# visinf/irr

Measured on AMD Instinct MI355X. Metric: image-pairs/sec fwd+bwd IRR-PWC 384x448 bs32, higher is better.
Workload: dtype f32 (fp16x2 split operands)

## Files before the change

### irr_amd/csrc/conv_x3.hip

```cpp
#include "x3_split.h"
#include "pack.h"
#include "amax.h"
#include <stdlib.h>
#include <atomic>

#ifdef X3S_TRACE
static unsigned long long* g_x3s_dbg = nullptr;
#endif

#ifndef X3_ABL
#define X3_ABL 0
#endif

int irr_amax_channels_launch(const float* x, int B, int C, long hw, long bs, float* out, hipStream_t st, bool zero);

namespace {

constexpr uint32_t OOB = 0x80000000u;

struct X3Args {
  const float* x;
  const u32x4* wq;
  const float* bias;
  const float* res;
  float* y;
  int B, Cin, H, W, Cout;
  int dil;
  int RD;
  int CoT, nchunk;
  int TR, TC, tiles_x, tiles_y;
  long x_bs, y_bs, res_bs;
  int lrelu, accumulate;
  float alpha;
  const float* mask;
  long mask_bs;
  int nmask;
  int ngy;
  int ksplit;
  float* part;
  const float* x_amax;
  int n_amax;
  float* y_amax;
  float* y_chmax;
  unsigned int* kcnt;
};

template <int CT, int PG, int NT, int PLANE_PIX, int NP = 3>
__global__ __launch_bounds__(CT* PG * 64, 2) void conv_x3_kernel(const X3Args a) {
  constexpr int NTHR = CT * PG * 64;
  constexpr int NR = (2 * PLANE_PIX + NTHR - 1) / NTHR;
  __shared__ u32x4 lds[2 * NP * PLANE_PIX];

  const int tid = threadIdx.x;
  const int lane = tid & 63;
  const int wave = __builtin_amdgcn_readfirstlane(tid >> 6);
  const int ct = wave % CT, pg = wave / CT;
  const int j = lane & 31, g = lane >> 5;
  const unsigned xpos = irr_xcd_order(blockIdx.x, gridDim.x);
  const int by = (int)(xpos % (unsigned)a.ngy);
  int bt = (int)(xpos / (unsigned)a.ngy);
  const int tx = bt % a.tiles_x;
  bt /= a.tiles_x;
  const int ty = bt % a.tiles_y;
  bt /= a.tiles_y;
  const int rr = bt % a.RD;
  const int b = bt / a.RD;
  const int y0 = ty * a.TR, x0 = tx * a.TC;
  const int d = a.dil;
  const int dy = a.RD > 1 ? 1 : d;
  const int Hs = (a.H - rr + a.RD - 1) / a.RD;
  const int LW = a.TC + 2 * d, LH = a.TR + 2 * dy;
  const int npix = LH * LW;
  const long hw = (long)a.H * a.W;
  const int cot = by * CT + ct;
  const bool active = cot < a.CoT;

  const __amdgpu_buffer_rsrc_t xr = __builtin_amdgcn_make_buffer_rsrc((void*)a.x, (short)0, (int)0x80000000u, 0x00020000);
  const __amdgpu_buffer_rsrc_t wr = __builtin_amdgcn_make_buffer_rsrc((void*)a.wq, (short)0, (int)0xffffffffu, 0x00020000);

  uint32_t svoff[NR];
  int swidx[NR];
#pragma unroll
  for (int r = 0; r < NR; ++r) {
    const int u = r * NTHR + tid;
    const int gg = u >= npix ? 1 : 0;
    const int pix = u - gg * npix;
    const bool inr = u < 2 * npix;
    const int ly = pix / LW, lx = pix - ly * LW;
    const int iy = y0 - dy + ly, ix = x0 - d + lx;
    const bool ok = inr && iy >= 0 && iy < Hs && ix >= 0 && ix < a.W;
    svoff[r] = ok ? (uint32_t)(((long)b * a.x_bs + (long)gg * 8 * hw + (long)(rr + iy * a.RD) * a.W + ix) * 4) : OOB;
    swidx[r] = inr ? gg * PLANE_PIX + pix : -1;
  }
  const uint32_t hw4 = (uint32_t)(hw * 4);
  const int tail_base = a.Cin - 16;

  int xidx[NT];
#pragma unroll
  for (int s = 0; s < NT; ++s) {
    const int t = (pg * NT + s) * 32 + j;
    const int row = t / a.TC, col = t - row * a.TC;
    xidx[s] = g * PLANE_PIX + row * LW + col;
  }
  const uint32_t wvoff = (uint32_t)((cot * 64 + lane) * 16);
  const uint32_t wpiece = (uint32_t)a.CoT * 1024u;
  const uint32_t wtap = (uint32_t)NP * wpiece;
  float sx = 1.f, inv_x = 1.f, inv_w = 1.f;
  if (NP == 2) {
    const int ex = x3_h2_exp(x3_h2_amax(a.x_amax, a.n_amax));
    const int ew = ((const int*)(a.wq + (long)a.nchunk * 9 * NP * a.CoT * 64))[0];
    sx = ldexpf(1.f, ex);
    inv_x = ldexpf(1.f, -ex);
    inv_w = ldexpf(1.f, -ew);
  }

  f32x16 acc[NT];
#pragma unroll
  for (int s = 0; s < NT; ++s)
#pragma unroll
    for (int r = 0; r < 16; ++r) acc[s][r] = 0.f;

  float raw[NR][8];
  auto issue_x = [&](int c) {
    const int ch0 = X3_ABL == 12 ? 0 : (c == a.nchunk - 1) ? tail_base : c * 16;
    const uint32_t s0 = (uint32_t)ch0 * hw4;
#pragma unroll
    for (int r = 0; r < NR; ++r)
#pragma unroll
      for (int e = 0; e < 8; ++e)
        raw[r][e] = (X3_ABL == 3 && c > 0) ? 1.f : __builtin_bit_cast(float, __builtin_amdgcn_raw_buffer_load_b32(xr, (int)svoff[r], (int)(s0 + e * hw4), 0));
  };
  u32x4 wa[2][NP];
  auto issue_w = [&](int slot, int c, int tap) {
    const uint32_t so = ((uint32_t)c * 9u + (uint32_t)tap) * wtap;
#pragma unroll
    for (int p = 0; p < NP; ++p)
      wa[slot][p] = __builtin_bit_cast(u32x4, __builtin_amdgcn_raw_buffer_load_b128(wr, (int)wvoff, (int)(so + p * wpiece), 0));
  };
  const int c_begin = (int)(((long)blockIdx.z * a.nchunk) / a.ksplit), c_end = (int)(((long)(blockIdx.z + 1) * a.nchunk) / a.ksplit);
  if (active) issue_w(0, c_begin, 0);

  for (int c = c_begin; c < c_end; ++c) {
    issue_x(c);
#pragma unroll
    for (int r = 0; r < NR; ++r) {
      u32x4 h, m, l;
      if (NP == 2) split8_h2<true>(raw[r], sx, h, m);
      else split8(raw[r], h, m, l);
      if (swidx[r] >= 0) {
        lds[swidx[r]] = h;
        lds[swidx[r] + 2 * PLANE_PIX] = m;
        if (NP == 3) lds[swidx[r] + 4 * PLANE_PIX] = l;
      }
    }
    __syncthreads();
    const bool more = c + 1 < c_end;
    if (active) {
#pragma unroll
      for (int tap = 0; tap < 9; ++tap) {
        const int slot = tap & 1;
        if (X3_ABL != 1) {
          const int nt = tap == 8 ? 0 : tap + 1;
          const int nc = tap == 8 ? (more ? c + 1 : c) : c;
          issue_w(slot ^ 1, nc, nt);
        }
        __builtin_amdgcn_sched_barrier(0);
        const int toff = (tap / 3) * LW * dy + (tap % 3) * d;
        u32x4 wdn;
        if (NP == 2) wdn = h2_hi_down(wa[slot][0]);
        u32x4 xb[2][NP];
#pragma unroll
        for (int p = 0; p < NP; ++p) xb[0][p] = lds[xidx[0] + toff + 2 * p * PLANE_PIX];
#pragma unroll
        for (int s = 0; s < NT; ++s) {
          const int cur = s & 1;
          if (s + 1 < NT) {
#pragma unroll
            for (int p = 0; p < NP; ++p) xb[cur ^ 1][p] = lds[xidx[s + 1] + toff + 2 * p * PLANE_PIX];
          }
          __builtin_amdgcn_sched_barrier(0);
          f32x16 t = acc[s];
          if constexpr (NP == 2) {
            t = mma_h(wa[slot][1], xb[cur][0], t);
            t = mma_h(wdn, xb[cur][1], t);
            t = mma_h(wa[slot][0], xb[cur][0], t);
          } else {
            if (X3_ABL != 20) {
            t = mma(wa[slot][NP - 1], xb[cur][0], t);
            t = mma(wa[slot][0], xb[cur][NP - 1], t);
            t = mma(wa[slot][1], xb[cur][1], t);
            }
            t = mma(wa[slot][1], xb[cur][0], t);
            t = mma(wa[slot][0], xb[cur][1], t);
            t = mma(wa[slot][0], xb[cur][0], t);
          }
          acc[s] = t;
          __builtin_amdgcn_sched_barrier(0);
        }
      }
#pragma unroll
      for (int p = 0; p < NP; ++p) wa[0][p] = wa[1][p];
    }
    __syncthreads();
  }
  if constexpr (NT > 4) {
    if (!active) return;
  }
  if (active && NP == 2) {
#pragma unroll
    for (int s = 0; s < NT; ++s)
#pragma unroll
      for (int r = 0; r < 16; ++r) acc[s][r] = (acc[s][r] * inv_x) * inv_w;
  }
  const long ohw = hw;
  bool split_out = a.ksplit > 1;
  if constexpr (NT <= 4)
  if (a.ksplit > 1 && a.kcnt != nullptr) {
    if (active) {
#pragma unroll
      for (int s = 0; s < NT; ++s) {
        const int t = (pg * NT + s) * 32 + j;
        const int row = t / a.TC, col = t - row * a.TC;
        const int oys = y0 + row, ox = x0 + col;
        if (oys >= Hs || ox >= a.W) continue;
        float* pb = a.part + (((long)blockIdx.z * a.B + b) * a.Cout) * ohw + (long)(rr + oys * a.RD) * a.W + ox;
#pragma unroll
        for (int r = 0; r < 16; ++r) {
          const int co = cot * 32 + (r & 3) + 8 * (r >> 2) + 4 * g;
          if (co < a.Cout) __hip_atomic_store(pb + (long)co * ohw, acc[s][r], __ATOMIC_RELAXED, __HIP_MEMORY_SCOPE_AGENT);
        }
      }
    }
    __shared__ unsigned int s_last;
    asm volatile("s_waitcnt vmcnt(0)" ::: "memory");
    __syncthreads();
    if (tid == 0) {
      const unsigned int old = atomicInc(a.kcnt + blockIdx.x, (unsigned int)a.ksplit - 1u);
      s_last = old == (unsigned int)a.ksplit - 1u ? 1u : 0u;
    }
    __syncthreads();
    if (!s_last) return;
    if (active) {
#pragma unroll
      for (int s = 0; s < NT; ++s) {
        const int t = (pg * NT + s) * 32 + j;
        const int row = t / a.TC, col = t - row * a.TC;
        const int oys = y0 + row, ox = x0 + col;
        if (oys >= Hs || ox >= a.W) continue;
        const long pofs0 = ((long)b * a.Cout) * ohw + (long)(rr + oys * a.RD) * a.W + ox;
        const long kstride = (long)a.B * a.Cout * ohw;
        f32x16 sum;
#pragma unroll
        for (int r = 0; r < 16; ++r) sum[r] = 0.f;
        for (int k = 0; k < a.ksplit; ++k) {
          float tv[16];
#pragma unroll
          for (int r = 0; r < 16; ++r) {
            const int co = cot * 32 + (r & 3) + 8 * (r >> 2) + 4 * g;
            const int cc = co < a.Cout ? co : a.Cout - 1;
            tv[r] = __hip_atomic_load(a.part + pofs0 + (long)cc * ohw + (long)k * kstride, __ATOMIC_RELAXED, __HIP_MEMORY_SCOPE_AGENT);
          }
#pragma unroll
          for (int r = 0; r < 16; ++r) sum[r] += tv[r];
        }
        acc[s] = sum;
      }
    }
    split_out = false;
  }
  if (!active) return;
  float ymax = 0.f;
  const bool want_amax = NP == 2 && a.y_amax != nullptr && !split_out;
  const bool want_ch = NP == 2 && a.y_chmax != nullptr && !split_out;
  float chm[16];
#pragma unroll
  for (int r = 0; r < 16; ++r) chm[r] = 0.f;

  const __amdgpu_buffer_rsrc_t yr = __builtin_amdgcn_make_buffer_rsrc((void*)(a.y + (long)b * a.y_bs), (short)0, (int)0x80000000u, 0x00020000);
  const __amdgpu_buffer_rsrc_t rsr =
      __builtin_amdgcn_make_buffer_rsrc((void*)(a.res ? a.res + (long)b * a.res_bs : a.y), (short)0, (int)0x80000000u, 0x00020000);
  const __amdgpu_buffer_rsrc_t mkr =
      __builtin_amdgcn_make_buffer_rsrc((void*)(a.mask ? a.mask + (long)b * a.mask_bs : a.y), (short)0, (int)0x80000000u, 0x00020000);
#pragma unroll
  for (int s = 0; s < NT; ++s) {
    const int t = (pg * NT + s) * 32 + j;
    const int row = t / a.TC, col = t - row * a.TC;
    const int oys = y0 + row, ox = x0 + col;
    if (oys >= Hs || ox >= a.W) continue;
    const long pofs = (long)(rr + oys * a.RD) * a.W + ox;
    if (split_out) {
      float* pb = a.part + (((long)blockIdx.z * a.B + b) * a.Cout) * ohw + pofs;
#pragma unroll
      for (int r = 0; r < 16; ++r) {
        const int co = cot * 32 + (r & 3) + 8 * (r >> 2) + 4 * g;
        if (co < a.Cout) pb[(long)co * ohw] = acc[s][r];
      }
      continue;
    }
    constexpr int RB = NT >= 8 ? 8 : 16;
#pragma unroll
    for (int r0 = 0; r0 < 16; r0 += RB) {
      uint32_t vo[RB];
      float bv[RB];
#pragma unroll
      for (int k = 0; k < RB; ++k) {
        const int r = r0 + k;
        const int co = cot * 32 + (r & 3) + 8 * (r >> 2) + 4 * g;
        const bool ok = co < a.Cout;
        vo[k] = ok ? (uint32_t)(((long)co * ohw + pofs) * 4) : OOB;
        bv[k] = (ok && a.bias) ? a.bias[co] : 0.f;
      }
      if (!a.res && !a.accumulate && !a.mask) {
#pragma unroll
        for (int k = 0; k < RB; ++k) {
          float v = acc[s][r0 + k] + bv[k];
          if (a.lrelu) v = irr_lrelu(v);
          v *= a.alpha;
          if (want_ch) { if (vo[k] != OOB) chm[r0 + k] = x3_amax_fold(chm[r0 + k], v); }
          else if (want_amax && vo[k] != OOB) ymax = x3_amax_fold(ymax, v);
          __builtin_amdgcn_raw_buffer_store_b32(__builtin_bit_cast(uint32_t, v), yr, (int)vo[k], 0, 0);
        }
        continue;
      }
      float rv[RB], dv[RB], mv[RB];
#pragma unroll
      for (int k = 0; k < RB; ++k) {
        const int r = r0 + k;
        const int co = cot * 32 + (r & 3) + 8 * (r >> 2) + 4 * g;
        rv[k] = __builtin_bit_cast(float, __builtin_amdgcn_raw_buffer_load_b32(rsr, (int)(a.res ? vo[k] : OOB), 0, 0));
        dv[k] = __builtin_bit_cast(float, __builtin_amdgcn_raw_buffer_load_b32(yr, (int)(a.accumulate ? vo[k] : OOB), 0, 0));
        mv[k] = __builtin_bit_cast(float, __builtin_amdgcn_raw_buffer_load_b32(mkr, (int)((a.mask && co < a.nmask) ? vo[k] : OOB), 0, 0));
      }
#pragma unroll
      for (int k = 0; k < RB; ++k) {
        const int r = r0 + k;
        const int co = cot * 32 + (r & 3) + 8 * (r >> 2) + 4 * g;
        float v = acc[s][r] + bv[k];
        if (a.lrelu) v = irr_lrelu(v);
        v = a.res ? rv[k] + a.alpha * v : v * a.alpha;
        v += dv[k];
        if (a.mask && co < a.nmask) v *= irr_lrelu_grad(mv[k]);
        if (want_ch) { if (vo[k] != OOB) chm[r] = x3_amax_fold(chm[r], v); }
        else if (want_amax && vo[k] != OOB) ymax = x3_amax_fold(ymax, v);
        __builtin_amdgcn_raw_buffer_store_b32(__builtin_bit_cast(uint32_t, v), yr, (int)vo[k], 0, 0);
      }
    }
  }
  if (want_ch && want_amax) {
#pragma unroll
    for (int r = 0; r < 16; ++r) ymax = __builtin_bit_cast(float, max(__builtin_bit_cast(uint32_t, ymax), __builtin_bit_cast(uint32_t, chm[r])));
  }
  if (want_amax) x3_amax_publish(ymax, a.y_amax);
  if (want_ch) {
    uint32_t mine = 0u;
#pragma unroll
    for (int r = 0; r < 16; ++r) {
      const uint32_t mb = x3_amax_half_upper(__builtin_bit_cast(uint32_t, chm[r]));
      mine = j == 16 + r ? mb : mine;
    }
    if (j >= 16) {
      const int r = j - 16;
      const int co = cot * 32 + (r & 3) + 8 * (r >> 2) + 4 * g;
      if (co < a.Cout) x3_amax_commit(__builtin_bit_cast(float, mine), a.y_chmax + co);
    }
  }
}

static thread_local float* g_next_chmax = nullptr;
static std::atomic<int> g_min_blocks{384};

struct X3SArgs {
  const float* x;
  const u32x4* wq;
  const float* bias;
  const float* res;
  float* y;
  int B, Cin, H, W, Cout;
  int tiles_x, tiles_y;
  long ntiles;
  long x_bs, y_bs, res_bs;
  int lrelu, accumulate;
  float alpha;
  const float* mask;
  long mask_bs;
  int nmask;
  unsigned long long* dbg;
  int wCoT, wcot;
  float* y2;
  long y2_bs;
  const float* x_amax;
  int n_amax;
  float* y_amax;
  float* y_chmax;
  const uint32_t* mask_bits;
  uint32_t* bits_out;
  long bits_tile0;
};

#ifdef X3S_TRACE
#define TR(slot) do { if (blockIdx.x == 7 && lane == 0 && ntr < 400) { dbgp[ntr++] = ((unsigned long long)(slot) << 56) | (__builtin_amdgcn_s_memtime() & 0xffffffffffffffull); } } while (0)
#else
#define TR(slot) do {} while (0)
#endif

#ifndef X3S_PRODUCERS_OLD
#define X3S_PRODUCERS_OLD 1
#endif
template <int EPI, int NP = 3>
__global__ __launch_bounds__(512) void conv_x3s_kernel(const X3SArgs a) {
  constexpr int PLANE_PIX = 352;
  constexpr int CHUNK = 2 * NP * PLANE_PIX;
  constexpr int LW = 34;
  constexpr int WUNITS = 18 * NP * 64;
  extern __shared__ u32x4 lds[];
  u32x4* const wl = lds;
  u32x4* const xl = lds + WUNITS;
  float* const ol = (float*)(lds + WUNITS + 2 * CHUNK);

  const int tid = threadIdx.x;
  const int lane = tid & 63;
  const int wave = __builtin_amdgcn_readfirstlane(tid >> 6);
  const long hw = (long)a.H * a.W;
  const long t_begin = irr_xcd_order(blockIdx.x, gridDim.x), t_step = gridDim.x;
#ifdef X3S_TRACE
  int ntr = 0;
  unsigned long long* dbgp = a.dbg + (size_t)wave * 400;
#endif

  for (int u = tid; u < WUNITS; u += 512) wl[u] = a.wq[((long)(u >> 6) * a.wCoT + a.wcot) * 64 + (u & 63)];
  float sx = 1.f, inv_x = 1.f, inv_w = 1.f;
  if (NP == 2) {
    const int ex = x3_h2_exp(x3_h2_amax(a.x_amax, a.n_amax));
    const int ew = ((const int*)(a.wq + (long)18 * NP * a.wCoT * 64))[0];
    sx = ldexpf(1.f, ex);
    inv_x = ldexpf(1.f, -ex);
    inv_w = ldexpf(1.f, -ew);
  }
  __syncthreads();

  if (X3S_PRODUCERS_OLD ? wave < 4 : wave >= 4) {
    const int ptid = X3S_PRODUCERS_OLD ? tid : tid - 256;
    const __amdgpu_buffer_rsrc_t xr = __builtin_amdgcn_make_buffer_rsrc((void*)a.x, (short)0, (int)0x80000000u, 0x00020000);
    const __amdgpu_buffer_rsrc_t rres = __builtin_amdgcn_make_buffer_rsrc((void*)a.res, (short)0, (int)0x80000000u, 0x00020000);
    const __amdgpu_buffer_rsrc_t ry = __builtin_amdgcn_make_buffer_rsrc((void*)a.y, (short)0, (int)0x80000000u, 0x00020000);
    const __amdgpu_buffer_rsrc_t rmask = __builtin_amdgcn_make_buffer_rsrc((void*)a.mask, (short)0, (int)0x80000000u, 0x00020000);
    const __amdgpu_buffer_rsrc_t ry2 = __builtin_amdgcn_make_buffer_rsrc((void*)(EPI == 3 ? a.y2 : a.y), (short)0, (int)0x80000000u, 0x00020000);
    const __amdgpu_buffer_rsrc_t rbits = __builtin_amdgcn_make_buffer_rsrc((void*)(EPI == 4 ? (const void*)a.mask_bits : (const void*)a.bits_out),
                                                                            (short)0, (int)0x80000000u, 0x00020000);
    const int su_gg = ptid / 100, su_rest = ptid % 100;
    const int su_ly = su_rest / 10, su_q = su_rest % 10;
    const bool su_act = ptid < 200;
    const uint32_t hw4 = (uint32_t)(hw * 4);
    const uint32_t c1off = (uint32_t)(a.Cin - 16) * hw4;
    f32x4 raw[2][8];
    struct TileAt { int b, ty, tx; };
    const int step_x = (int)(t_step % a.tiles_x), step_y = (int)((t_step / a.tiles_x) % a.tiles_y),
              step_b = (int)(t_step / ((long)a.tiles_x * a.tiles_y));
    auto advance = [&](TileAt& c) {
      c.tx += step_x;
      const int cx = c.tx >= a.tiles_x;
      c.tx -= cx ? a.tiles_x : 0;
      c.ty += step_y + cx;
      const int cy = c.ty >= a.tiles_y;
      c.ty -= cy ? a.tiles_y : 0;
      c.b += step_b + cy;
    };
    auto issue_chunk = [&](const TileAt& at, int c, bool valid) {
      const int tx = X3_ABL == 11 ? 1 : at.tx, ty = X3_ABL == 11 ? 1 : at.ty, b = X3_ABL == 11 ? 0 : at.b;
      const int iy = ty * 8 - 1 + su_ly, ix = tx * 32 - 4 + su_q * 4;
      const bool ok = valid && su_act && iy >= 0 && iy < a.H && ix >= 0 && ix < a.W && X3_ABL != 10;
      const uint32_t vo = ok ? (uint32_t)(((long)b * a.x_bs + (long)su_gg * 8 * hw + (long)iy * a.W + ix) * 4) : OOB;
#pragma unroll
      for (int e = 0; e < 8; ++e)
        raw[c][e] = __builtin_bit_cast(f32x4, __builtin_amdgcn_raw_buffer_load_b128(xr, (int)vo, (int)((c ? c1off : 0u) + e * hw4), 0));
    };
    auto write_chunk = [&](int c) {
      u32x4* buf = xl + c * CHUNK + su_gg * PLANE_PIX + su_ly * LW;
#pragma unroll
      for (int px = 0; px < 4; ++px) {
        const int lx = su_q * 4 + px - 3;
        float v[8];
#pragma unroll
        for (int e = 0; e < 8; ++e) v[e] = raw[c][e][px];
        u32x4 h, m, l;
        if (NP == 2) split8_h2<true>(v, sx, h, m);
        else split8(v, h, m, l);
        if (su_act && lx >= 0 && lx < LW) {
          buf[lx] = h;
          buf[lx + 2 * PLANE_PIX] = m;
          if (NP == 3) buf[lx + 4 * PLANE_PIX] = l;
        }
      }
    };
    const int eq_q = ptid & 7, eq_row = (ptid >> 3) & 7, eq_c8 = ptid >> 6;
    float bias_r[8];
#pragma unroll
    for (int e = 0; e < 8; ++e) bias_r[e] = (a.bias && eq_c8 * 8 + e < a.Cout) ? a.bias[eq_c8 * 8 + e] : 0.f;
    f32x4 erv[8], edv[8], emv[8];
    uint32_t evd = OOB, evd2 = OOB;
    uint32_t ebits = 0, ebo = OOB;
    auto epilogue_loads = [&](const TileAt& at, bool valid, long tix) {
      const int tx = at.tx, ty = at.ty, b = at.b;
      const int oy = ty * 8 + eq_row, ox = tx * 32 + eq_q * 4;
      const bool pv = valid && oy < a.H && ox < a.W;
      const long pofs = (long)oy * a.W + ox + (long)eq_c8 * 8 * hw;
      const uint32_t vr = (EPI >= 1 && pv && a.res) ? (uint32_t)(((long)b * a.res_bs + pofs) * 4) : OOB;
// ... 786 lines not shown
```

Before: 211.6.

## Double-buffer LDS input planes and interleave next-chunk loads with MFMA taps

Adds a pipelined path for the fp16x2 (NP==2), large-NT conv_x3 configurations. The LDS input plane is double-buffered, and loading, splitting and storing the next channel chunk are spread across the tap/subtile MFMA loop. This removes one barrier per chunk and hides the global load latency behind compute. Weight prefetch deepens to three slots, two taps ahead. The cost is double the LDS footprint and more live registers, which may lower occupancy or cause spills.

```diff
diff --git a/irr_amd/csrc/conv_x3.hip b/irr_amd/csrc/conv_x3.hip
--- a/irr_amd/csrc/conv_x3.hip
+++ b/irr_amd/csrc/conv_x3.hip
@@ -10,6 +10,9 @@
 
 #ifndef X3_ABL
 #define X3_ABL 0
+#endif
+#ifndef X3_PIPE
+#define X3_PIPE 1
 #endif
 
 int irr_amax_channels_launch(const float* x, int B, int C, long hw, long bs, float* out, hipStream_t st, bool zero);
@@ -49,7 +52,9 @@
 __global__ __launch_bounds__(CT* PG * 64, 2) void conv_x3_kernel(const X3Args a) {
   constexpr int NTHR = CT * PG * 64;
   constexpr int NR = (2 * PLANE_PIX + NTHR - 1) / NTHR;
-  __shared__ u32x4 lds[2 * NP * PLANE_PIX];
+  constexpr bool PIPE = X3_PIPE && X3_ABL != 13 && NP == 2 && NT >= 7 && NR <= 5;
+  constexpr int BUF = 2 * NP * PLANE_PIX;
+  __shared__ u32x4 lds[(PIPE ? 2 : 1) * BUF];
 
   const int tid = threadIdx.x;
   const int lane = tid & 63;
@@ -138,9 +143,112 @@
       wa[slot][p] = __builtin_bit_cast(u32x4, __builtin_amdgcn_raw_buffer_load_b128(wr, (int)wvoff, (int)(so + p * wpiece), 0));
   };
   const int c_begin = (int)(((long)blockIdx.z * a.nchunk) / a.ksplit), c_end = (int)(((long)(blockIdx.z + 1) * a.nchunk) / a.ksplit);
-  if (active) issue_w(0, c_begin, 0);
-
+  if (active && !PIPE) issue_w(0, c_begin, 0);
+
+  if constexpr (PIPE) {
+    constexpr auto XI = [](int r) { return NR <= 3 ? 3 * r : 2 * r; };
+    constexpr int XK = NR <= 3 ? 3 : 2;
+    u32x4 wp[3][NP];
+    auto issue_wp = [&](int slot, int c, int tap) {
+      const uint32_t so = ((uint32_t)c * 9u + (uint32_t)tap) * wtap;
+#pragma unroll
+      for (int p = 0; p < NP; ++p)
+        wp[slot][p] = __builtin_bit_cast(u32x4, __builtin_amdgcn_raw_buffer_load_b128(wr, (int)wvoff, (int)(so + p * wpiece), 0));
+    };
+    auto issue_round = [&](float (&v)[8], int c, int r, bool valid) {
+      const int ch0 = X3_ABL == 12 ? 0 : (c == a.nchunk - 1) ? tail_base : c * 16;
+      const uint32_t s0 = (uint32_t)ch0 * hw4;
+      const uint32_t vo = valid ? svoff[r] : OOB;
+#pragma unroll
+      for (int e = 0; e < 8; ++e)
+        v[e] = __builtin_bit_cast(float, __builtin_amdgcn_raw_buffer_load_b32(xr, (int)vo, (int)(s0 + e * hw4), 0));
+    };
+    auto write_round = [&](const u32x4& h, const u32x4& m, int r, int base) {
+      if (swidx[r] >= 0) {
+        lds[base + swidx[r]] = h;
+        lds[base + swidx[r] + 2 * PLANE_PIX] = m;
+      }
+    };
+    issue_x(c_begin);
+#pragma unroll
+    for (int r = 0; r < NR; ++r) {
+      u32x4 h, m;
+      split8_h2<true>(raw[r], sx, h, m);
+      write_round(h, m, r, 0);
+    }
+    __syncthreads();
+    if (!active) {
+      for (int c = c_begin; c + 1 < c_end; ++c) {
+        const int wb = ((c - c_begin) & 1) ? 0 : BUF;
+#pragma unroll
+        for (int r = 0; r < NR; ++r) {
+          float v[8];
+          u32x4 h, m;
+          issue_round(v, c + 1, r, true);
+          split8_h2<true>(v, sx, h, m);
+          write_round(h, m, r, wb);
+        }
+        __syncthreads();
+      }
+      return;
+    }
+    issue_wp(0, c_begin, 0);
+    issue_wp(1, c_begin, 1);
+    float v[8];
+    u32x4 sh, sm;
+    for (int c = c_begin; c < c_end; ++c) {
+      const bool more = c + 1 < c_end;
+      const int rb = ((c - c_begin) & 1) ? BUF : 0;
+      const int wb = BUF - rb;
+      const int cn = more ? c + 1 : c;
+#pragma unroll
+      for (int tap = 0; tap < 9; ++tap) {
+        const int slot = tap % 3;
+        if (X3_ABL != 1) {
+          const int nt = tap + 2 > 8 ? tap + 2 - 9 : tap + 2;
+          const int nc = tap + 2 > 8 ? (more ? c + 1 : c) : c;
+          issue_wp((tap + 2) % 3, nc, nt);
+        }
+        __builtin_amdgcn_sched_barrier(0);
+        const int toff = rb + (tap / 3) * LW * dy + (tap % 3) * d;
+        u32x4 wdn = h2_hi_down(wp[slot][0]);
+        u32x4 xb[2][NP];
+#pragma unroll
+        for (int p = 0; p < NP; ++p) xb[0][p] = lds[xidx[0] + toff + 2 * p * PLANE_PIX];
+#pragma unroll
+        for (int s = 0; s < NT; ++s) {
+          const int cur = s & 1;
+          if (s + 1 < NT) {
+#pragma unroll
+            for (int p = 0; p < NP; ++p) xb[cur ^ 1][p] = lds[xidx[s + 1] + toff + 2 * p * PLANE_PIX];
+          }
+          __builtin_amdgcn_sched_barrier(0);
+          f32x16 t = acc[s];
+          t = mma_h(wp[slot][1], xb[cur][0], t);
+          t = mma_h(wdn, xb[cur][1], t);
+          t = mma_h(wp[slot][0], xb[cur][0], t);
+          acc[s] = t;
+#pragma unroll
+          for (int r = 0; r < NR; ++r) {
+            if (s == 0 && XI(r) + XK == tap) split8_h2<true>(v, sx, sh, sm);
+            if (s == 0 && XI(r) == tap) issue_round(v, cn, r, more);
+            if (s == 1 && XI(r) + XK == tap) write_round(sh, sm, r, wb);
+          }
+          __builtin_amdgcn_sched_barrier(0);
+        }
+      }
+#pragma unroll
+      for (int r = 0; r < NR; ++r) {
+        if (XI(r) + XK > 8) {
+          split8_h2<true>(v, sx, sh, sm);
+          write_round(sh, sm, r, wb);
+        }
+      }
+      __syncthreads();
+    }
+  } else
   for (int c = c_begin; c < c_end; ++c) {
+    if (X3_ABL != 13 || c == c_begin) {
     issue_x(c);
 #pragma unroll
     for (int r = 0; r < NR; ++r) {
@@ -154,6 +262,7 @@
       }
     }
     __syncthreads();
+    }
     const bool more = c + 1 < c_end;
     if (active) {
 #pragma unroll
@@ -201,7 +310,7 @@
 #pragma unroll
       for (int p = 0; p < NP; ++p) wa[0][p] = wa[1][p];
     }
-    __syncthreads();
+    if (X3_ABL != 13) __syncthreads();
   }
   if constexpr (NT > 4) {
     if (!active) return;
```

Result: faster. 213.8, median of 6 (+1.1%).
